# yuanzhi-zhu/DiffPIR

Measured on AMD Instinct MI355X. Metric: restored images/sec @100 NFE, 256x256, higher is better.
Workload: dtype f32 (GEMMs as 3 x f16 MFMA on hi/lo-split fp32 operands, fp32 accumulate; exact-fp32-MFMA mode in alt_precision); 1 GPU; configs[1]: ffhq topology 256x256 deblur (61x61 Gaussian PSF), 100 NFE, batch 16/GPU, device Philox noise, hipGraph=on; global_batch=16, nfe=100, collective=none

## Files before the change

diffpir_amd/_lib.py:

```python
from __future__ import annotations

import ctypes as C
import os

_HERE = os.path.dirname(os.path.abspath(__file__))
LIB_PATH = os.environ.get("DIFFPIR_LIB") or os.path.join(_HERE, "csrc", "libdiffpir_hip.so")
ABI_VERSION = 2



class UNetDesc(C.Structure):
    _fields_ = [("image_size", C.c_int32), ("in_channels", C.c_int32), ("model_channels", C.c_int32),
                ("out_channels", C.c_int32), ("num_res_blocks", C.c_int32), ("num_head_channels", C.c_int32),
                ("n_channel_mult", C.c_int32), ("channel_mult", C.c_float * 8),
                ("n_attention_ds", C.c_int32), ("attention_ds", C.c_int32 * 8), ("num_classes", C.c_int32)]


class Tensor(C.Structure):
    _fields_ = [("name", C.c_char_p), ("data", C.c_void_p), ("ndim", C.c_int32), ("shape", C.c_int64 * 4)]


class Step(C.Structure):
    _fields_ = [("t", C.c_int32), ("last", C.c_int32), ("c1", C.c_float), ("c2", C.c_float), ("tau", C.c_float),
                ("sa_t", C.c_float), ("s1m_t", C.c_float), ("sa_p", C.c_float),
# ... 164 lines not shown

DEBUG_LIB_PATH = os.path.join(_HERE, "csrc", "libdiffpir_dbg.so")
_dbg = None


def load_debug():
    global _dbg
    if _dbg is not None:
        return _dbg
    load()
    if not os.path.exists(DEBUG_LIB_PATH):
        raise EngineLibraryError(f"{DEBUG_LIB_PATH} not found: `make -C diffpir_amd/csrc` builds it next to the product library")
    d = C.CDLL(DEBUG_LIB_PATH)
    d.dpir_debug_conv_bench.argtypes = [C.c_void_p] + [C.c_int] * 10 + [C.POINTER(C.c_double)]
    d.dpir_debug_conv7_emit_supported.argtypes = [C.c_void_p] + [C.c_int] * 4 + [C.POINTER(C.c_int)]
    d.dpir_debug_victim.argtypes = [C.c_void_p, C.c_int, C.c_int, C.c_int, C.c_longlong, C.c_int, C.POINTER(C.c_ulonglong)]
    d.dpir_debug_victim_alu.argtypes = [C.c_void_p, C.c_int, C.c_int, C.c_int, C.c_int, C.POINTER(C.c_ulonglong)]
    for fn in (d.dpir_debug_victim_fft_pk, d.dpir_debug_victim_fft_nopk):
        fn.argtypes = [C.c_void_p, C.c_int, C.c_int, C.c_int, C.POINTER(C.c_ulonglong)]
    d.dpir_debug_conv7_check.argtypes = [C.c_void_p] + [C.c_int] * 10 + [C.POINTER(C.c_double), C.POINTER(C.c_double), C.POINTER(C.c_ulonglong),
                                                                        C.POINTER(C.c_float), C.POINTER(C.c_int)]
    d.dpir_debug_conv5_layer.argtypes = [C.c_void_p] + [C.c_int] * 7 + [C.c_void_p] * 7 + [C.POINTER(C.c_int)]
    d.dpir_debug_conv5_layer.restype = C.c_int
    d.dpir_debug_conv3_layer.argtypes = [C.c_void_p, C.POINTER(Conv3Desc)]
    d.dpir_debug_conv3_layer.restype = C.c_int
    d.dpir_debug_conv9_layer.argtypes = [C.c_void_p, C.POINTER(Conv9Desc)]
    d.dpir_debug_conv9_layer.restype = C.c_int
    d.dpir_debug_conv_up_layer.argtypes = [C.c_void_p, C.POINTER(ConvUpDesc)]
    d.dpir_debug_conv_up_layer.restype = C.c_int
    d.dpir_debug_conv_up_counts.argtypes = [C.POINTER(C.c_longlong), C.POINTER(C.c_longlong)]
    d.dpir_debug_conv_up_counts.restype = None
    d.dpir_debug_attention.argtypes = [C.c_void_p, C.POINTER(AttentionDesc)]
    d.dpir_debug_attention.restype = C.c_int
    d.dpir_debug_groupnorm.argtypes = [C.c_void_p, C.POINTER(GroupNormDesc)]
    d.dpir_debug_groupnorm.restype = C.c_int
    for n in ("dpir_debug_conv_bench", "dpir_debug_victim", "dpir_debug_victim_alu", "dpir_debug_victim_fft_pk", "dpir_debug_victim_fft_nopk",
              "dpir_debug_conv7_check"):
        getattr(d, n).restype = C.c_int
    _dbg = d
    return d


def load():
    global _lib
    if _lib is not None:
        return _lib
# ... 24 lines not shown
```

diffpir_amd/csrc/common.h:

```cpp
#pragma once
#include <hip/hip_runtime.h>
#include <stdint.h>
#include <stdio.h>
#include <string>
#include <vector>
#include <map>
#include <memory>
#include <mutex>

#include "../../include/diffpir_engine.h"

namespace dpir {

struct Status {
    int code = DPIR_OK;
    std::string msg;
    bool ok() const { return code == DPIR_OK; }
};

#define DPIR_HIP(expr)                                                                         \
    do {                                                                                       \
        hipError_t _e = (expr);                                                                \
        if (_e != hipSuccess) {                                                                \
            char _b[512];                                                                      \
// ... 126 lines not shown
    const struct Conv6Emit* emit = nullptr;
};
bool conv7_emit_supported(int B, int Cout, int H, int W);
bool conv6_supported(int H, int W);
int conv6_stat_slots(int H, int W);
Status launch_conv6(hipStream_t s, const Conv6Args& a, int* stat_kind_out = nullptr, PendingConv* pend_out = nullptr, int* kernel_out = nullptr);
Status launch_conv6_resolve(hipStream_t s, const PendingConv& p);
float pack_weights_conv6(const float* w_oihw, int cout, int cin, std::vector<uint16_t>& out);
struct Conv5Args {
    CatSrc src; const float4* prm = nullptr;
    const void* w16 = nullptr; float w16_scale = 1.f;
    const float* bias = nullptr; float* out = nullptr; const float* res = nullptr;
    int B = 0, Cout = 0, H = 0, W = 0;
    unsigned long long* range_ctr = nullptr;
    bool x1 = false;
    const float4* emit_prm = nullptr; void* emit_hi = nullptr; void* emit_lo = nullptr;
    const float* out_scale_dev = nullptr;
    int force_tile = 0;
};
constexpr int kConv5EmitMaxC = 384;
bool conv5_supported(int B, int Cout, int H, int W, bool has_prm = false);
bool conv5_small_supported(int B, int ca, int cb, int Cout, int H, int W, bool has_prm = false);
Status launch_conv5(hipStream_t s, const Conv5Args& a);
float pack_weights_f16x3_1x1(const float* w_oi, int cout, int cin, std::vector<uint16_t>& out);
struct Conv8Args {
    const float* x = nullptr;
    const float4* prm = nullptr;
    const void* w = nullptr; float w_scale = 1.f;
    const float* bias = nullptr; float* out = nullptr;
    int B = 0, C = 0, Cout = 0, H = 0, W = 0;
    unsigned long long* range_ctr = nullptr;
    bool x1 = false;
    bool silu = true;
};
bool conv8_supported(int B, int C, int Cout, int H, int W);
Status launch_conv8(hipStream_t s, const Conv8Args& a);
float pack_weights_conv8(const float* w_oihw, int cout, int cin, std::vector<uint16_t>& out);
Status launch_gn_stats(hipStream_t s, CatSrc src, int B, int HW, double2* part);
struct GnStatSrc { const float2* slots = nullptr; int nslots = 0; const double2* part = nullptr; int c = 0; };
Status launch_gn_prm(hipStream_t s, GnStatSrc sa, GnStatSrc sb, int HW, const float* gamma, const float* beta,
                     const float* film, int film_stride, int film_off, int B, int C, bool silu, float4* prm,
                     const StepDev* fstep = nullptr, int frows = 0, float2* stats_out = nullptr);
Status launch_time_embed(hipStream_t s, const int* t_dev, const int* y_dev, const float* freqs, const float* w0, const float* b0,
                         const float* w2, const float* b2, const float* label_emb, int B, int mc, float* tmp, float* semb);
Status launch_rows_gemv(hipStream_t s, const float* W, const float* bias, const float* x, int B, int R, int K, float* out);

// ... 4 lines not shown
```

diffpir_amd/csrc/conv5.hip:

```cpp
#include "common.h"
#include "lds_dma.h"
#include <vector>
#include <stdlib.h>

namespace dpir {

typedef float floatx16 __attribute__((ext_vector_type(16)));
typedef _Float16 half8 __attribute__((ext_vector_type(8)));

struct Conv5K {
    const float* sa; const float* sb; int ca, cb;
    unsigned bytes_a, bytes_b, bytes_w, bytes_prm;
    const float4* prm;
    const char* w16; const float* bias; float* out; const float* res;
    int B, Cout, HW;
    int n_chunks, n_co_blocks;
    int n_wblocks;
    int n_tiles, pair_xcd;
    long long total_px;
    float out_scale;
    const float* out_scale_dev;
    unsigned long long* range_ctr;
    const float4* eprm; _Float16* ehi; _Float16* elo; int eC8;
};


__device__ __forceinline__ float gn_apply(float v, const float4 m, bool silu) {
    float t = (v - m.x) * m.y + m.z;
    if (silu) t = t * __builtin_amdgcn_rcpf(1.0f + __builtin_amdgcn_exp2f(t * -1.4426950408889634f));
    return t;
}

template <bool HAS_PRM, bool X1, bool EMIT, int WCO, int WPX, int TPX>
__device__ __forceinline__ bool conv5_chunk(const float* __restrict__ xs, const half8* __restrict__ wh, const float4* __restrict__ ps,
                                            const float4* __restrict__ eprm, const int (&pxl)[WPX], const int (&pimg)[WPX], bool silu, bool emit_wg,
                                            _Float16* __restrict__ ehi, _Float16* __restrict__ elo, const size_t (&eoff)[WPX], size_t echunk,
                                            floatx16 (&acc)[WCO][WPX]) {
    const half8* wl = wh + 2 * (32 * WCO);
    bool bad = false;
    half8 bh[WPX], bl[WPX];
#pragma unroll
    for (int j = 0; j < WPX; ++j) {
        float v[8];
#pragma unroll
        for (int jj = 0; jj < 8; ++jj) v[jj] = xs[jj * TPX + pxl[j]];
        if (HAS_PRM) {
#pragma unroll
            for (int jj = 0; jj < 8; ++jj) v[jj] = gn_apply(v[jj], ps[pimg[j] * 16 + jj], silu);
        }
        if (EMIT) {
            if (emit_wg) {
                half8 eh, el;
#pragma unroll
                for (int jj = 0; jj < 8; ++jj) {
                    float t = gn_apply(v[jj], eprm[jj], silu);
                    bad |= !(fabsf(t) <= 65000.f);
                    t = fminf(fmaxf(t, -65000.f), 65000.f);
                    const _Float16 hh = (_Float16)t;
                    eh[jj] = hh;
                    el[jj] = (_Float16)(t - (float)hh);
                }
                const size_t eo = (eoff[j] + echunk) * 8;
                *reinterpret_cast<half8*>(ehi + eo) = eh;
                if (!X1) *reinterpret_cast<half8*>(elo + eo) = el;
            }
        }
#pragma unroll
        for (int jj = 0; jj < 8; ++jj) {
            bad |= !(fabsf(v[jj]) <= 65000.f);
            float x = fminf(fmaxf(v[jj], -65000.f), 65000.f);
            _Float16 hh = (_Float16)x;
            bh[j][jj] = hh;
            if (!X1) bl[j][jj] = (_Float16)(x - (float)hh);
        }
    }
    half8 ah[WCO], al[WCO];
#pragma unroll
    for (int i = 0; i < WCO; ++i) { ah[i] = wh[i * 32]; if (!X1) al[i] = wl[i * 32]; }
    if (!X1) {
#pragma unroll
        for (int i = 0; i < WCO; ++i)
#pragma unroll
            for (int j = 0; j < WPX; ++j)
                acc[i][j] = __builtin_amdgcn_mfma_f32_32x32x16_f16(al[i], bh[j], acc[i][j], 0, 0, 0);
#pragma unroll
        for (int i = 0; i < WCO; ++i)
#pragma unroll
            for (int j = 0; j < WPX; ++j)
                acc[i][j] = __builtin_amdgcn_mfma_f32_32x32x16_f16(ah[i], bl[j], acc[i][j], 0, 0, 0);
    }
#pragma unroll
    for (int i = 0; i < WCO; ++i)
#pragma unroll
        for (int j = 0; j < WPX; ++j)
            acc[i][j] = __builtin_amdgcn_mfma_f32_32x32x16_f16(ah[i], bh[j], acc[i][j], 0, 0, 0);
    return bad;
}

template <bool HAS_PRM, bool X1, bool EMIT, int WCO, int WPX, int NST>
__device__ __forceinline__ void conv5_body(const Conv5K p) {
    static_assert(!(HAS_PRM && EMIT), "the emitting variant multiplies the raw input");
    static_assert(!EMIT || (WCO == 4 && WPX == 2 && NST == 3), "planes are emitted by the 128 x 256 tile only");
    static_assert((WPX == 1 || WPX == 2) && (WCO == 2 || WCO == 4) && NST >= 3 && NST <= 4, "tile / ring shapes the DMA split is written for");
#if defined(__HIP_DEVICE_COMPILE__)
    constexpr int TCO = 32 * WCO, TPX = 128 * WPX;
    constexpr int XBYTES = 16 * TPX * 4;
    constexpr int WBYTES = TCO * 64;
    constexpr int PBYTES = HAS_PRM ? 1024 : 0;
    constexpr int STAGE = XBYTES + WBYTES + PBYTES;
    constexpr int NSTORE = EMIT ? (X1 ? WPX : 2 * WPX) : 0;
    __shared__ __attribute__((aligned(16))) char smem5[NST * STAGE + 512 + (EMIT ? kConv5EmitMaxC * 16 : 0)];
    float* bias_sh = reinterpret_cast<float*>(smem5 + NST * STAGE);
    float4* eprm_sh = reinterpret_cast<float4*>(smem5 + NST * STAGE + 512);

    const int tid = threadIdx.x;
    const int lane = tid & 63;
    const int wave = __builtin_amdgcn_readfirstlane(tid >> 6);
    const int l31 = lane & 31;
    const int half = lane >> 5;
    const int bid = blockIdx.x;
    int co_blk, tile;
    if (p.pair_xcd) {
        const int t = bid >> 3;
        co_blk = t % p.n_co_blocks;
// ... 10 lines not shown
    const int n_tile = px0 / HW;
    const bool emit_wg = EMIT && co_blk == 0;
    const bool prm_wave = HAS_PRM && wave == 0;

    const __amdgpu_buffer_rsrc_t rs_a = rsrc_uniform(p.sa, p.bytes_a);
    const __amdgpu_buffer_rsrc_t rs_b = rsrc_uniform(p.sb ? p.sb : p.sa, p.sb ? p.bytes_b : 0u);
    const __amdgpu_buffer_rsrc_t rs_w = rsrc_uniform(p.w16, p.bytes_w);
    const __amdgpu_buffer_rsrc_t rs_p = rsrc_uniform(HAS_PRM ? (const void*)p.prm : (const void*)p.w16, HAS_PRM ? p.bytes_prm : 0u);
    constexpr int RPI = 256 / TPX, LPR = 64 / RPI;
    constexpr int XPW = 4 / RPI;
    constexpr int WPW = WBYTES / 1024 / 4;
    const int lr = lane / LPR;
    const int gq = px0 + 4 * (lane % LPR);
    const bool q_ok = gq < total_px;
    const int qn = q_ok ? gq / HW : 0;
    const int qp = q_ok ? gq - qn * HW : 0;
    const unsigned voffA = q_ok ? (unsigned)(((size_t)qn * p.ca * HW + (size_t)lr * HW + qp) * 4) : kOutOfRange;
    const unsigned voffB = q_ok ? (unsigned)(((size_t)qn * p.cb * HW + (size_t)lr * HW + qp) * 4) : kOutOfRange;
    const unsigned lane16 = (unsigned)lane * 16u;
    const unsigned voffP = (HAS_PRM && n_tile + (lane >> 4) < p.B) ? (unsigned)(((size_t)(n_tile + (lane >> 4)) * C + (lane & 15)) * 16) : kOutOfRange;

    auto issue_dma = [&](int chunk, int st) __attribute__((always_inline)) {
        char* stage = smem5 + st * STAGE;
#pragma unroll
        for (int u = 0; u < XPW; ++u) {
            const int cc = wave * XPW + u;
            const int c = chunk * 16 + cc * RPI;
            char* dst = stage + cc * 1024;
            if (c < p.ca) BLDS6(rs_a, dst, (RPI == 1 || c + lr < p.ca) ? voffA : kOutOfRange, (unsigned)c * (unsigned)HW * 4u);
            else BLDS6(rs_b, dst, c + lr < C ? voffB : kOutOfRange, (unsigned)(c - p.ca) * (unsigned)HW * 4u);
        }
        constexpr int WPLANE = TCO * 16;
        const unsigned wsoff = TCO == 128 ? (unsigned)(chunk * p.n_co_blocks + co_blk) * 8192u
                                          : (unsigned)(chunk * p.n_wblocks + (co_blk >> 1)) * 8192u + (unsigned)(co_blk & 1) * (unsigned)WPLANE;
#pragma unroll
        for (int u = 0; u < WPW; ++u) {
            const int piece = wave * WPW + u;
            const int pb = piece * 1024;
            BLDS6(rs_w, stage + XBYTES + pb, lane16 + (pb / WPLANE) * 2048 + pb % WPLANE, wsoff);
        }
        if (prm_wave) BLDS6(rs_p, stage + XBYTES + WBYTES, voffP, (unsigned)chunk * 256u);
    };

    int pxl[WPX]; int pimg[WPX];
    size_t eoff[WPX];
#pragma unroll
    for (int j = 0; j < WPX; ++j) {
        pxl[j] = wave * (32 * WPX) + j * 32 + l31;
        const int g = px0 + pxl[j];
        const int pn = g < total_px ? g / HW : n_tile;
        pimg[j] = pn - n_tile;
        eoff[j] = EMIT ? ((size_t)pn * p.eC8 + half) * HW + (size_t)(g - pn * HW) : 0;
    }

    floatx16 acc[WCO][WPX];
#pragma unroll
    for (int i = 0; i < WCO; ++i)
#pragma unroll
        for (int j = 0; j < WPX; ++j)
#pragma unroll
            for (int r = 0; r < 16; ++r) acc[i][j][r] = 0.f;

    bool bad = false;
    bool silu = false;
    if (EMIT) {
        for (int c = tid; c < C; c += 256) eprm_sh[c] = p.eprm[(size_t)n_tile * C + c];
        silu = __builtin_amdgcn_readfirstlane(p.eprm[0].w != 0.f ? 1 : 0) != 0;
    }
    if (HAS_PRM) silu = __builtin_amdgcn_readfirstlane(p.prm[0].w != 0.f ? 1 : 0) != 0;
    if (tid < TCO) bias_sh[tid] = co_blk * TCO + tid < p.Cout ? p.bias[co_blk * TCO + tid] : 0.f;
    __builtin_amdgcn_sched_barrier(0);
    issue_dma(0, 0);
    if (p.n_chunks > 1) issue_dma(1, 1);
    if (NST > 3 && p.n_chunks > 2) issue_dma(2, 2);
    int st = 0;
    for (int chunk = 0; chunk < p.n_chunks; ++chunk) {
        constexpr int NDMA = XPW + WPW;
        __builtin_amdgcn_sched_barrier(0);
        if (chunk + 1 >= p.n_chunks) wait_vmcnt<0>();
        else if (NST > 3 && chunk + 2 < p.n_chunks) { if (prm_wave) wait_vmcnt<2 * NDMA + 2>(); else wait_vmcnt<2 * NDMA>(); }
        else if (emit_wg && chunk > 0) wait_vmcnt<NDMA + NSTORE>();
        else if (prm_wave) wait_vmcnt<NDMA + 1>();
        else wait_vmcnt<NDMA>();
        barrier_lds_only();
        if (chunk + NST - 1 < p.n_chunks) issue_dma(chunk + NST - 1, st == 0 ? NST - 1 : st - 1);
        __builtin_amdgcn_sched_barrier(0);

        const char* stage = smem5 + st * STAGE;
        bad |= conv5_chunk<HAS_PRM, X1, EMIT, WCO, WPX, TPX>(reinterpret_cast<const float*>(stage) + (8 * half) * TPX,
                                              reinterpret_cast<const half8*>(stage + XBYTES) + half * TCO + l31,
                                              reinterpret_cast<const float4*>(stage + XBYTES + WBYTES) + 8 * half,
                                              eprm_sh + chunk * 16 + 8 * half, pxl, pimg, silu, emit_wg,
                                              p.ehi, p.elo, eoff, (size_t)chunk * 2 * HW, acc);
        st = st == NST - 1 ? 0 : st + 1;
    }

    {
        const unsigned long long m = __ballot(bad);
        if (m != 0ull && p.range_ctr && lane == __builtin_ctzll(m)) atomicAdd(p.range_ctr, (unsigned long long)__builtin_popcountll(m));
    }
    __syncthreads();
    constexpr int SROW = 32 * WPX + 4;
    static_assert(4 * 32 * SROW * 4 <= NST * STAGE, "epilogue slabs alias the ring");
    constexpr int L4 = 8 * WPX;
    constexpr int NPS = 32 / (64 / L4);
    float* slab = reinterpret_cast<float*>(smem5) + wave * (32 * SROW);
    const int row_l = lane / L4, c4 = lane % L4;
    const int g4 = px0 + wave * (32 * WPX) + 4 * c4;
    const bool ok4 = g4 < total_px;
    const int n4 = ok4 ? g4 / HW : 0;
    const size_t base4 = (size_t)n4 * p.Cout * HW + (size_t)(g4 - n4 * HW);
    const int co0 = co_blk * TCO;
    const float osc = p.out_scale_dev ? p.out_scale * p.out_scale_dev[0] : p.out_scale;
#pragma unroll
    for (int i = 0; i < WCO; ++i) {
#pragma unroll
        for (int j = 0; j < WPX; ++j)
// ... 9 lines not shown
            }
            wait_vmcnt<0>();
        }
#pragma unroll
        for (int ps = 0; ps < NPS; ++ps) {
            const int row = ps * (64 / L4) + row_l;
            const int co = co0 + i * 32 + row;
            const float4 a4 = *reinterpret_cast<const float4*>(slab + row * SROW + 4 * c4);
            const float bz = bias_sh[i * 32 + row];
            if (ok4 && co < p.Cout) {
                float4 v = make_float4(a4.x * osc + bz, a4.y * osc + bz, a4.z * osc + bz, a4.w * osc + bz);
                if (p.res) v = make_float4(rr[ps].x + v.x, rr[ps].y + v.y, rr[ps].z + v.z, rr[ps].w + v.w);
                *reinterpret_cast<float4*>(p.out + base4 + (size_t)co * HW) = v;
            }
        }
    }
#endif
}

template <bool HAS_PRM, bool X1, bool EMIT>
__global__ __launch_bounds__(256, 2) void conv5_mfma_kernel(Conv5K p) { conv5_body<HAS_PRM, X1, EMIT, 4, 2, 3>(p); }
template <bool HAS_PRM, bool X1>
__global__ __launch_bounds__(256, 2) void conv5_small_mfma_kernel(Conv5K p) { conv5_body<HAS_PRM, X1, false, 2, 1, 4>(p); }

static bool conv5_shape_ok(int H, int W, bool has_prm) {
    if ((H * W) % 4) return false;
    return !(has_prm && (H * W) % 64);
}

bool conv5_supported(int B, int Cout, int H, int W, bool has_prm) {
    const long long px = (long long)B * H * W;
    if (!conv5_shape_ok(H, W, has_prm)) return false;
    return ((px + 255) / 256) * ((Cout + 127) / 128) >= 32;
}

static bool conv5_small_enabled() {
    static const bool on = !(getenv("DPIR_CONV5_SMALL") && atoi(getenv("DPIR_CONV5_SMALL")) == 0);
    return on;
}
static long long conv5_small_below() {
    static const long long v = getenv("DPIR_CONV5_SMALL_BELOW") ? atoll(getenv("DPIR_CONV5_SMALL_BELOW")) : 512;
    return v;
}
static bool conv5_small_shape_ok(int ca, int cb, int H, int W, bool has_prm) {
    return conv5_shape_ok(H, W, has_prm) && !(cb > 0 && ca % 4);
}

bool conv5_small_supported(int B, int ca, int cb, int Cout, int H, int W, bool has_prm) {
    const long long px = (long long)B * H * W;
    if (!conv5_small_enabled() || !conv5_small_shape_ok(ca, cb, H, W, has_prm)) return false;
    if (((px + 255) / 256) * ((Cout + 127) / 128) >= conv5_small_below()) return false;
    return ((px + 127) / 128) * ((Cout + 63) / 64) >= 32;
}

Status launch_conv5(hipStream_t s, const Conv5Args& a) {
    const int ca = a.src.ca, cb = a.src.b ? a.src.cb : 0;
    const bool has_prm = a.prm != nullptr;
    bool small;
    if (a.force_tile) {
        small = a.force_tile == 2;
        if (small ? (!conv5_small_shape_ok(ca, cb, a.H, a.W, has_prm) || a.emit_hi) : !conv5_shape_ok(a.H, a.W, has_prm))
            return Status{DPIR_ERR_UNSUPPORTED, "conv5: shape not tiled"};
    } else {
        small = !a.emit_hi && conv5_small_supported(a.B, ca, cb, a.Cout, a.H, a.W, has_prm);
        if (!small && !conv5_supported(a.B, a.Cout, a.H, a.W, has_prm)) return Status{DPIR_ERR_UNSUPPORTED, "conv5: shape not tiled"};
// ... 9 lines not shown
    k.n_wblocks = (a.Cout + 127) / 128;
    k.total_px = (long long)a.B * a.H * a.W;
    if (k.total_px >= (1ll << 31) - 256) return invalid("conv5: more than 2^31 pixels in the batch");
    const unsigned long long ba = (unsigned long long)k.total_px * k.ca * 4, bb = (unsigned long long)k.total_px * k.cb * 4;
    const unsigned long long bw = (unsigned long long)k.n_chunks * k.n_wblocks * 8192, bp = (unsigned long long)a.B * C * 16;
    if (ba >= (1ull << 32) || bb >= (1ull << 32) || bw >= (1ull << 32))
        return invalid("conv5: an input tensor exceeds the 4 GiB buffer-descriptor range; reduce the batch");
    k.bytes_a = (unsigned)ba; k.bytes_b = (unsigned)bb; k.bytes_w = (unsigned)bw; k.bytes_prm = (unsigned)bp;
    if (a.prm && C % 16) return invalid("conv5: the GroupNorm variant needs a multiple of 16 input channels");
    k.out_scale = 1.0f / a.w16_scale;
    k.out_scale_dev = a.out_scale_dev;
    k.range_ctr = a.range_ctr;
    k.eprm = a.emit_prm; k.ehi = reinterpret_cast<_Float16*>(a.emit_hi); k.elo = reinterpret_cast<_Float16*>(a.emit_lo);
    k.eC8 = 2 * k.n_chunks;
    k.n_tiles = (int)((k.total_px + tpx - 1) / tpx);
    static const bool pair_env = !(getenv("DPIR_CONV5_PAIR") && atoi(getenv("DPIR_CONV5_PAIR")) == 0);
    k.pair_xcd = pair_env && k.n_co_blocks > 1 ? 1 : 0;
    const unsigned blocks = k.pair_xcd ? (unsigned)((k.n_tiles + 7) / 8 * 8 * k.n_co_blocks) : (unsigned)(k.n_tiles * k.n_co_blocks);
    if (a.emit_hi) {
        if (a.prm || !a.emit_prm || (!a.x1 && !a.emit_lo)) return invalid("conv5: the plane-emitting variant takes the raw input and a GroupNorm table for the planes");
        if ((a.H * a.W) % 256 || C % 16 || C > kConv5EmitMaxC) return invalid("conv5: the plane-emitting variant needs H*W % 256 == 0 and a multiple of 16, at most 384, input channels");
        if (a.x1) hipLaunchKernelGGL((conv5_mfma_kernel<false, true, true>), dim3(blocks), dim3(256), 0, s, k);
        else hipLaunchKernelGGL((conv5_mfma_kernel<false, false, true>), dim3(blocks), dim3(256), 0, s, k);
    } else if (small) {
        if (a.x1) {
            if (a.prm) hipLaunchKernelGGL((conv5_small_mfma_kernel<true, true>), dim3(blocks), dim3(256), 0, s, k);
            else hipLaunchKernelGGL((conv5_small_mfma_kernel<false, true>), dim3(blocks), dim3(256), 0, s, k);
        } else if (a.prm) hipLaunchKernelGGL((conv5_small_mfma_kernel<true, false>), dim3(blocks), dim3(256), 0, s, k);
        else hipLaunchKernelGGL((conv5_small_mfma_kernel<false, false>), dim3(blocks), dim3(256), 0, s, k);
    } else if (a.x1) {
        if (a.prm) hipLaunchKernelGGL((conv5_mfma_kernel<true, true, false>), dim3(blocks), dim3(256), 0, s, k);
        else hipLaunchKernelGGL((conv5_mfma_kernel<false, true, false>), dim3(blocks), dim3(256), 0, s, k);
    } else if (a.prm) hipLaunchKernelGGL((conv5_mfma_kernel<true, false, false>), dim3(blocks), dim3(256), 0, s, k);
    else hipLaunchKernelGGL((conv5_mfma_kernel<false, false, false>), dim3(blocks), dim3(256), 0, s, k);
    DPIR_HIP(hipGetLastError());
    return Status{};
}

float pack_weights_f16x3_1x1(const float* w, int cout, int cin, std::vector<uint16_t>& out) {
    const int chunks = (cin + 15) / 16, cblocks = (cout + 127) / 128;
    float mx = 0.f;
    for (size_t i = 0; i < (size_t)cout * cin; ++i) mx = fmaxf(mx, fabsf(w[i]));
    float scale = 1.0f;
    if (mx > 0.f) scale = exp2f(floorf(log2f(1024.0f / mx)));
    while (mx * scale >= 1024.0f) scale *= 0.5f;
    const size_t plane = (size_t)2 * 128 * 8;
// ... 22 lines not shown
```

diffpir_amd/csrc/dbg_conv.hip:

```cpp
#include "engine.h"
#include "conv6_params.h"
#include "conv9.h"
#include "conv_up.h"
#include "../../include/diffpir_debug.h"
#include <string.h>
#include <vector>
using namespace dpir;
static int fail(dpir_engine* e, const Status& s) {
    if (e) e->last_error = s.msg;
    return s.code;
}
#define API_TRY(e, expr)                          \
    do {                                          \
        Status _s = (expr);                       \
        if (!_s.ok()) return fail((e), _s);       \
    } while (0)
#define API_HIP(e, expr)                                                                  \
    do {                                                                                  \
        hipError_t _h = (expr);                                                           \
        if (_h != hipSuccess)                                                             \
            return fail((e), Status{DPIR_ERR_HIP, std::string(#expr) + ": " + hipGetErrorString(_h)}); \
    } while (0)

__global__ void dbg_bitdiff_kernel(const float* a, const float* b, size_t n, unsigned long long* out) {
// ... 171 lines not shown
    }
    unsigned long long h[2] = {0, 0};
    API_HIP(e, hipMemcpyAsync(h, cmp, 16, hipMemcpyDeviceToHost, e->stream));
    API_HIP(e, hipStreamSynchronize(e->stream));
    *mismatches_out = h[0];
    const unsigned mb = (unsigned)h[1];
    *maxdiff_out = __builtin_bit_cast(float, mb);
    hipEvent_t e0, e1, e2;
    API_HIP(e, hipEventCreate(&e0)); API_HIP(e, hipEventCreate(&e1)); API_HIP(e, hipEventCreate(&e2));
    for (int i = 0; i < 3; ++i) { API_TRY(e, launch_conv6(e->stream, a6, &k6, &pend)); API_TRY(e, launch_conv7(e->stream, k, blocks * S, x1 != 0)); }
    API_HIP(e, hipEventRecord(e0, e->stream));
    for (int i = 0; i < iters; ++i) API_TRY(e, launch_conv6(e->stream, a6, &k6, &pend));
    API_HIP(e, hipEventRecord(e1, e->stream));
    for (int i = 0; i < iters; ++i) API_TRY(e, launch_conv7(e->stream, k, blocks * S, x1 != 0));
    API_HIP(e, hipEventRecord(e2, e->stream));
    API_HIP(e, hipEventSynchronize(e2));
    float m6 = 0, m7 = 0;
    API_HIP(e, hipEventElapsedTime(&m6, e0, e1)); API_HIP(e, hipEventElapsedTime(&m7, e1, e2));
    (void)hipEventDestroy(e0); (void)hipEventDestroy(e1); (void)hipEventDestroy(e2);
    *ms6_out = m6 / iters; *ms7_out = m7 / iters;
    return DPIR_OK;
}

int dpir_debug_conv5_layer(dpir_engine* e, int B, int ca, int cb, int Cout, int H, int W, int tile, const float* xa, const float* xb,
                           const float* w, const float* bias, const float* prm, const float* res, float* out, int* path_out) {
    if (!e || !xa || !w || !bias || !out || !path_out || B <= 0 || ca <= 0 || cb < 0 || (cb > 0 && !xb) || Cout <= 0 || tile < 0 || tile > 2) return DPIR_ERR_INVALID;
    if (e->precision == 0) return fail(e, invalid("conv5 layer: the engine is in f32 mode"));
    (void)hipSetDevice(e->device);
    const int C = ca + cb, HW = H * W;
    const size_t na = (size_t)B * ca * HW, nb = (size_t)B * cb * HW, no = (size_t)B * Cout * HW;
    float *dxa = nullptr, *dxb = nullptr, *dbias = nullptr, *dout = nullptr, *dres = nullptr, *dw = nullptr, *partial = nullptr; float4* dprm = nullptr;
    API_TRY(e, e->ws.getT("c5#xa", na, &dxa));
    API_TRY(e, e->ws.getT("c5#xb", nb + 1, &dxb));
    API_TRY(e, e->ws.getT("c5#b", (size_t)round_up(Cout, 64), &dbias));
    API_TRY(e, e->ws.getT("c5#o", no, &dout));
    API_TRY(e, e->ws.getT("c5#res", no, &dres));
    API_TRY(e, e->ws.getT("c5#prm", (size_t)B * C, &dprm));
    API_HIP(e, hipMemcpy(dxa, xa, na * 4, hipMemcpyHostToDevice));
    if (cb) API_HIP(e, hipMemcpy(dxb, xb, nb * 4, hipMemcpyHostToDevice));
    API_HIP(e, hipMemset(dbias, 0, (size_t)round_up(Cout, 64) * 4));
    API_HIP(e, hipMemcpy(dbias, bias, (size_t)Cout * 4, hipMemcpyHostToDevice));
    if (prm) API_HIP(e, hipMemcpy(dprm, prm, (size_t)B * C * 16, hipMemcpyHostToDevice));
    if (res) API_HIP(e, hipMemcpy(dres, res, no * 4, hipMemcpyHostToDevice));
    API_HIP(e, hipMemset(dout, 0xFF, no * 4));
    std::vector<uint16_t> w16v;
    const float w16_scale = pack_weights_f16x3_1x1(w, Cout, C, w16v);
    void* wp = nullptr;
    API_TRY(e, e->ws.get("c5#w16", w16v.size() * 2, &wp));
    API_HIP(e, hipMemcpy(wp, w16v.data(), w16v.size() * 2, hipMemcpyHostToDevice));
    const bool has_prm = prm != nullptr;
    const bool use5 = !(has_prm && C % 16) && (tile != 0 || conv5_supported(B, Cout, H, W, has_prm) || conv5_small_supported(B, ca, cb, Cout, H, W, has_prm));
    Status st;
    if (use5) {
        Conv5Args a5;
        a5.src = CatSrc{dxa, ca, cb ? dxb : nullptr, cb}; a5.prm = has_prm ? dprm : nullptr; a5.w16 = wp; a5.w16_scale = w16_scale;
        a5.bias = dbias; a5.out = dout; a5.res = res ? dres : nullptr; a5.B = B; a5.Cout = Cout; a5.H = H; a5.W = W;
        a5.x1 = e->precision == 2; a5.force_tile = tile;
        *path_out = tile ? tile : (conv5_small_supported(B, ca, cb, Cout, H, W, has_prm) ? 2 : 1);
        st = launch_conv5(e->stream, a5);
    } else {
        const int coutp = round_up(Cout, 64), cinp = round_up(C, 16);
        std::vector<float> packed((size_t)cinp * coutp, 0.f);
        for (int co = 0; co < Cout; ++co)
            for (int ci = 0; ci < C; ++ci) packed[(size_t)ci * coutp + co] = w[(size_t)co * C + ci];
        API_TRY(e, e->ws.getT("c5#w", packed.size(), &dw));
        API_HIP(e, hipMemcpy(dw, packed.data(), packed.size() * 4, hipMemcpyHostToDevice));
        API_TRY(e, e->ws.getT("conv#partial", (size_t)16 * 1024 * 1024, &partial));
        ConvArgs a;
        a.src.a = dxa; a.src.ca = ca; a.src.b = cb ? dxb : nullptr; a.src.cb = cb; a.src.Hs = H; a.src.Ws = W; a.src.mode = 0;
        a.src.prm = has_prm ? dprm : nullptr;
        a.w = dw; a.bias = dbias; a.out = dout; a.res = res ? dres : nullptr; a.res_mode = 0;
        a.B = B; a.Cin = C; a.Cout = Cout; a.CoutP = coutp; a.H = H; a.W = W; a.ks = 1;
        a.partial = partial; a.partial_capacity = (size_t)16 * 1024 * 1024;
        *path_out = 0;
        st = launch_conv(e->stream, a);
    }
    API_TRY(e, st);
    API_HIP(e, hipStreamSynchronize(e->stream));
    API_HIP(e, hipMemcpy(out, dout, no * 4, hipMemcpyDeviceToHost));
    return DPIR_OK;
}

int dpir_debug_conv3_layer(dpir_engine* e, dpir_debug_conv3_desc* d) {
    if (!e || !d) return DPIR_ERR_INVALID;
    d->path_out = -1; d->ksplit_out = 0; d->stat_kind_out = 0;
    const int B = d->B, ca = d->ca, cb = d->cb, Cout = d->Cout, H = d->H, W = d->W, mode = d->mode, C = ca + cb;
    if (!d->xa || !d->w || !d->bias || !d->out || B <= 0 || ca <= 0 || cb < 0 || (cb > 0 && !d->xb) || Cout <= 0 || H <= 0 || W <= 0 || mode < 0 || mode > 2 ||
        d->res_mode < -1 || d->res_mode > 2 || (d->res_mode >= 0 && !d->res) || d->prologue < 0 || d->prologue > 2 ||
        (d->route != 0 && d->route != 6 && d->route != 7 && d->route != 8))
        return fail(e, invalid("conv3 layer: bad descriptor"));
    if (d->prologue == 1 && !d->prm) return fail(e, invalid("conv3 layer: prologue 1 needs the table"));
    if (d->prologue == 2 && (!d->gamma || !d->beta)) return fail(e, invalid("conv3 layer: prologue 2 needs gamma and beta"));
    if (mode == 1 && ((H | W) & 1)) return fail(e, invalid("conv3 layer: a nearest-up source needs an even output size"));
    if (d->res_mode == 1 && ((H | W) & 1)) return fail(e, invalid("conv3 layer: a half-resolution residual needs an even output size"));
    if (d->defer && (!d->split || (d->route != 0 && d->route != 7) || !d->gamma2 || !d->beta2 || !d->w2 || !d->bias2 || !d->out2 || d->Cout2 <= 0))
        return fail(e, invalid("conv3 layer: defer needs split, route 0 or 7 and the second stage's operands"));
    (void)hipSetDevice(e->device);
    const int Hs = mode == 1 ? H / 2 : (mode == 2 ? H * 2 : H), Ws = mode == 1 ? W / 2 : (mode == 2 ? W * 2 : W);
    const size_t HWs = (size_t)Hs * Ws, HW = (size_t)H * W;
    const size_t na = (size_t)B * ca * HWs, nb = (size_t)B * cb * HWs, no = (size_t)B * Cout * HW;
    const size_t nres = d->res_mode == 1 ? no / 4 : (d->res_mode == 2 ? no * 4 : no);
    const int coutp = round_up(Cout, 64);
// ... 444 lines not shown
```

include/diffpir_debug.h:

```cpp
#ifndef DIFFPIR_DEBUG_H
#define DIFFPIR_DEBUG_H
#include "diffpir_engine.h"
#ifdef __cplusplus
extern "C" {
#endif
int dpir_debug_conv_bench(dpir_engine* e, int B, int Cin, int Cout, int H, int W, int ks, int mode, int with_prm,
                          int dbg, int iters, double* ms_out);
int dpir_debug_victim(dpir_engine* e, int lds_bytes, int threads, int blocks, long long spin_ticks, int iters, unsigned long long* bad_out);
int dpir_debug_victim_alu(dpir_engine* e, int mode, int blocks, int iters_in_kernel, int launches, unsigned long long* bad_out);
int dpir_debug_victim_fft_pk(dpir_engine* e, int blocks, int iters_in_kernel, int launches, unsigned long long* bad_out);
int dpir_debug_victim_fft_nopk(dpir_engine* e, int blocks, int iters_in_kernel, int launches, unsigned long long* bad_out);
int dpir_debug_conv7_check(dpir_engine* e, int B, int Cin, int Cout, int H, int W, int res_mode, int x1, int split, int scaled, int iters,
                           double* ms6_out, double* ms7_out, unsigned long long* mismatches_out, float* maxdiff_out, int* ksplit_out);
int dpir_debug_conv7_emit_supported(dpir_engine* e, int B, int Cout, int H, int W, int* capacity_out);
int dpir_debug_conv5_layer(dpir_engine* e, int B, int ca, int cb, int Cout, int H, int W, int tile, const float* xa, const float* xb,
                           const float* w, const float* bias, const float* prm, const float* res, float* out, int* path_out);
typedef struct dpir_debug_conv3_desc {
    int32_t B, ca, cb, Cout, H, W, mode, res_mode, scaled, prologue, route, split, defer, Cout2;
    const float *xa, *xb, *w, *bias, *res, *prm, *gamma, *beta, *film, *gamma2, *beta2, *w2, *bias2;
    float* out; double* stat_out; float* out2;
    int32_t stat_kind_out, path_out, ksplit_out, reserved;
} dpir_debug_conv3_desc;
int dpir_debug_conv3_layer(dpir_engine* e, dpir_debug_conv3_desc* d);
typedef struct dpir_debug_conv9_desc {
    int32_t B, Cin, Cout, H, W, res_mode, hop, Cout2;
    const float *x, *w, *bias, *res, *prm, *gamma2, *beta2, *film2, *w2, *bias2;
    float* out; double* stat_out; float* out2;
    int32_t ran_out, iters;
    double ms_out;
} dpir_debug_conv9_desc;
int dpir_debug_conv9_layer(dpir_engine* e, dpir_debug_conv9_desc* d);
typedef struct dpir_debug_conv_up_desc {
    int32_t B, Cin, Cout, Hs, Ws, hop, force_hop, Cout2, route, reserved;
    const float *x, *w, *bias, *res, *prm, *gamma2, *beta2, *film2, *w2, *bias2;
    float* out; double* stat_out; float* out2;
    int32_t ran_out, iters;
    double ms_out;
} dpir_debug_conv_up_desc;
int dpir_debug_conv_up_layer(dpir_engine* e, dpir_debug_conv_up_desc* d);
// ... 21 lines not shown
```

Before: 9.150 images/s.

## Add software-pipelined conv5 small-tile kernel overlapping MFMA with next chunk's split

Adds a pipelined variant of the small-tile (2x1, 4-stage) conv5 kernel. It keeps four DMA stages in flight and double-buffers the f16 hi/lo operands, so the MFMAs for the current chunk run while the next chunk's LDS loads and hi/lo split are in progress. Interleaving is guided by sched_group_barrier. It also simplifies DMA address computation when channels align to 16, and it is on by default for eligible shapes. In exchange, register pressure is higher and the schedule is more complex; env and debug overrides allow falling back.

```diff
diff --git a/diffpir_amd/_lib.py b/diffpir_amd/_lib.py
--- a/diffpir_amd/_lib.py
+++ b/diffpir_amd/_lib.py
@@ -210,6 +210,10 @@
                                                                         C.POINTER(C.c_float), C.POINTER(C.c_int)]
     d.dpir_debug_conv5_layer.argtypes = [C.c_void_p] + [C.c_int] * 7 + [C.c_void_p] * 7 + [C.POINTER(C.c_int)]
     d.dpir_debug_conv5_layer.restype = C.c_int
+    d.dpir_debug_conv5_layer_range.argtypes = d.dpir_debug_conv5_layer.argtypes + [C.POINTER(C.c_ulonglong)]
+    d.dpir_debug_conv5_layer_range.restype = C.c_int
+    d.dpir_debug_set_conv5_small_pipe.argtypes = [C.c_int]
+    d.dpir_debug_set_conv5_small_pipe.restype = C.c_int
     d.dpir_debug_conv3_layer.argtypes = [C.c_void_p, C.POINTER(Conv3Desc)]
     d.dpir_debug_conv3_layer.restype = C.c_int
     d.dpir_debug_conv9_layer.argtypes = [C.c_void_p, C.POINTER(Conv9Desc)]
diff --git a/diffpir_amd/csrc/common.h b/diffpir_amd/csrc/common.h
--- a/diffpir_amd/csrc/common.h
+++ b/diffpir_amd/csrc/common.h
@@ -172,6 +172,7 @@
 bool conv5_supported(int B, int Cout, int H, int W, bool has_prm = false);
 bool conv5_small_supported(int B, int ca, int cb, int Cout, int H, int W, bool has_prm = false);
 Status launch_conv5(hipStream_t s, const Conv5Args& a);
+void conv5_small_pipe_override(int v);
 float pack_weights_f16x3_1x1(const float* w_oi, int cout, int cin, std::vector<uint16_t>& out);
 struct Conv8Args {
     const float* x = nullptr;
diff --git a/diffpir_amd/csrc/conv5.hip b/diffpir_amd/csrc/conv5.hip
--- a/diffpir_amd/csrc/conv5.hip
+++ b/diffpir_amd/csrc/conv5.hip
@@ -1,5 +1,6 @@
 #include "common.h"
 #include "lds_dma.h"
+#include <type_traits>
 #include <vector>
 #include <stdlib.h>
 
@@ -31,75 +32,98 @@
     return t;
 }
 
+template <int TPX>
+__device__ __forceinline__ void conv5_load_b(const float* __restrict__ xs, int pxl, float (&v)[8]) {
+#pragma unroll
+    for (int jj = 0; jj < 8; ++jj) v[jj] = xs[jj * TPX + pxl];
+}
+
+template <bool HAS_PRM, bool X1, bool EMIT>
+__device__ __forceinline__ bool conv5_split(float (&v)[8], const float4* __restrict__ ps, const float4* __restrict__ eprm, int pimg, bool silu, bool emit_wg,
+                                            _Float16* __restrict__ ehi, _Float16* __restrict__ elo, size_t eo, half8& bh, half8& bl) {
+    bool bad = false;
+    if (HAS_PRM) {
+#pragma unroll
+        for (int jj = 0; jj < 8; ++jj) v[jj] = gn_apply(v[jj], ps[pimg * 16 + jj], silu);
+    }
+    if (EMIT) {
+        if (emit_wg) {
+            half8 eh, el;
+#pragma unroll
+            for (int jj = 0; jj < 8; ++jj) {
+                float t = gn_apply(v[jj], eprm[jj], silu);
+                bad |= !(fabsf(t) <= 65000.f);
+                t = fminf(fmaxf(t, -65000.f), 65000.f);
+                const _Float16 hh = (_Float16)t;
+                eh[jj] = hh;
+                el[jj] = (_Float16)(t - (float)hh);
+            }
+            *reinterpret_cast<half8*>(ehi + eo) = eh;
+            if (!X1) *reinterpret_cast<half8*>(elo + eo) = el;
+        }
+    }
+#pragma unroll
+    for (int jj = 0; jj < 8; ++jj) {
+        bad |= !(fabsf(v[jj]) <= 65000.f);
+        float x = fminf(fmaxf(v[jj], -65000.f), 65000.f);
+        _Float16 hh = (_Float16)x;
+        bh[jj] = hh;
+        if (!X1) bl[jj] = (_Float16)(x - (float)hh);
+    }
+    return bad;
+}
+
+template <bool X1, int WCO>
+__device__ __forceinline__ void conv5_load_a(const half8* __restrict__ wh, half8 (&ah)[WCO], half8 (&al)[WCO]) {
+    const half8* wl = wh + 2 * (32 * WCO);
+#pragma unroll
+    for (int i = 0; i < WCO; ++i) { ah[i] = wh[i * 32]; if (!X1) al[i] = wl[i * 32]; }
+}
+
+template <bool X1, int WCO, int WPX>
+__device__ __forceinline__ void conv5_multiply(const half8 (&bh)[WPX], const half8 (&bl)[WPX], const half8 (&ah)[WCO], const half8 (&al)[WCO],
+                                               floatx16 (&acc)[WCO][WPX]) {
+    if (!X1) {
+#pragma unroll
+        for (int i = 0; i < WCO; ++i)
+#pragma unroll
+            for (int j = 0; j < WPX; ++j)
+                acc[i][j] = __builtin_amdgcn_mfma_f32_32x32x16_f16(al[i], bh[j], acc[i][j], 0, 0, 0);
+#pragma unroll
+        for (int i = 0; i < WCO; ++i)
+#pragma unroll
+            for (int j = 0; j < WPX; ++j)
+                acc[i][j] = __builtin_amdgcn_mfma_f32_32x32x16_f16(ah[i], bl[j], acc[i][j], 0, 0, 0);
+    }
+#pragma unroll
+    for (int i = 0; i < WCO; ++i)
+#pragma unroll
+        for (int j = 0; j < WPX; ++j)
+            acc[i][j] = __builtin_amdgcn_mfma_f32_32x32x16_f16(ah[i], bh[j], acc[i][j], 0, 0, 0);
+}
+
 template <bool HAS_PRM, bool X1, bool EMIT, int WCO, int WPX, int TPX>
 __device__ __forceinline__ bool conv5_chunk(const float* __restrict__ xs, const half8* __restrict__ wh, const float4* __restrict__ ps,
                                             const float4* __restrict__ eprm, const int (&pxl)[WPX], const int (&pimg)[WPX], bool silu, bool emit_wg,
                                             _Float16* __restrict__ ehi, _Float16* __restrict__ elo, const size_t (&eoff)[WPX], size_t echunk,
                                             floatx16 (&acc)[WCO][WPX]) {
-    const half8* wl = wh + 2 * (32 * WCO);
     bool bad = false;
-    half8 bh[WPX], bl[WPX];
+    half8 bh[WPX], bl[WPX], ah[WCO], al[WCO];
 #pragma unroll
     for (int j = 0; j < WPX; ++j) {
         float v[8];
-#pragma unroll
-        for (int jj = 0; jj < 8; ++jj) v[jj] = xs[jj * TPX + pxl[j]];
-        if (HAS_PRM) {
-#pragma unroll
-            for (int jj = 0; jj < 8; ++jj) v[jj] = gn_apply(v[jj], ps[pimg[j] * 16 + jj], silu);
-        }
-        if (EMIT) {
-            if (emit_wg) {
-                half8 eh, el;
-#pragma unroll
-                for (int jj = 0; jj < 8; ++jj) {
-                    float t = gn_apply(v[jj], eprm[jj], silu);
-                    bad |= !(fabsf(t) <= 65000.f);
-                    t = fminf(fmaxf(t, -65000.f), 65000.f);
-                    const _Float16 hh = (_Float16)t;
-                    eh[jj] = hh;
-                    el[jj] = (_Float16)(t - (float)hh);
-                }
-                const size_t eo = (eoff[j] + echunk) * 8;
-                *reinterpret_cast<half8*>(ehi + eo) = eh;
-                if (!X1) *reinterpret_cast<half8*>(elo + eo) = el;
-            }
-        }
-#pragma unroll
-        for (int jj = 0; jj < 8; ++jj) {
-            bad |= !(fabsf(v[jj]) <= 65000.f);
-            float x = fminf(fmaxf(v[jj], -65000.f), 65000.f);
-            _Float16 hh = (_Float16)x;
-            bh[j][jj] = hh;
-            if (!X1) bl[j][jj] = (_Float16)(x - (float)hh);
-        }
-    }
-    half8 ah[WCO], al[WCO];
-#pragma unroll
-    for (int i = 0; i < WCO; ++i) { ah[i] = wh[i * 32]; if (!X1) al[i] = wl[i * 32]; }
-    if (!X1) {
-#pragma unroll
-        for (int i = 0; i < WCO; ++i)
-#pragma unroll
-            for (int j = 0; j < WPX; ++j)
-                acc[i][j] = __builtin_amdgcn_mfma_f32_32x32x16_f16(al[i], bh[j], acc[i][j], 0, 0, 0);
-#pragma unroll
-        for (int i = 0; i < WCO; ++i)
-#pragma unroll
-            for (int j = 0; j < WPX; ++j)
-                acc[i][j] = __builtin_amdgcn_mfma_f32_32x32x16_f16(ah[i], bl[j], acc[i][j], 0, 0, 0);
-    }
-#pragma unroll
-    for (int i = 0; i < WCO; ++i)
-#pragma unroll
-        for (int j = 0; j < WPX; ++j)
-            acc[i][j] = __builtin_amdgcn_mfma_f32_32x32x16_f16(ah[i], bh[j], acc[i][j], 0, 0, 0);
+        conv5_load_b<TPX>(xs, pxl[j], v);
+        bad |= conv5_split<HAS_PRM, X1, EMIT>(v, ps, eprm, pimg[j], silu, emit_wg, ehi, elo, (eoff[j] + echunk) * 8, bh[j], bl[j]);
+    }
+    conv5_load_a<X1, WCO>(wh, ah, al);
+    conv5_multiply<X1, WCO, WPX>(bh, bl, ah, al, acc);
     return bad;
 }
 
-template <bool HAS_PRM, bool X1, bool EMIT, int WCO, int WPX, int NST>
+template <bool HAS_PRM, bool X1, bool EMIT, int WCO, int WPX, int NST, bool PIPE = false>
 __device__ __forceinline__ void conv5_body(const Conv5K p) {
     static_assert(!(HAS_PRM && EMIT), "the emitting variant multiplies the raw input");
+    static_assert(!PIPE || (!EMIT && WCO == 2 && WPX == 1 && NST == 4), "the pipelined loop is written for the small tile");
     static_assert(!EMIT || (WCO == 4 && WPX == 2 && NST == 3), "planes are emitted by the 128 x 256 tile only");
     static_assert((WPX == 1 || WPX == 2) && (WCO == 2 || WCO == 4) && NST >= 3 && NST <= 4, "tile / ring shapes the DMA split is written for");
 #if defined(__HIP_DEVICE_COMPILE__)
@@ -156,13 +180,23 @@
 
     auto issue_dma = [&](int chunk, int st) __attribute__((always_inline)) {
         char* stage = smem5 + st * STAGE;
-#pragma unroll
-        for (int u = 0; u < XPW; ++u) {
-            const int cc = wave * XPW + u;
-            const int c = chunk * 16 + cc * RPI;
-            char* dst = stage + cc * 1024;
-            if (c < p.ca) BLDS6(rs_a, dst, (RPI == 1 || c + lr < p.ca) ? voffA : kOutOfRange, (unsigned)c * (unsigned)HW * 4u);
-            else BLDS6(rs_b, dst, c + lr < C ? voffB : kOutOfRange, (unsigned)(c - p.ca) * (unsigned)HW * 4u);
+        if constexpr (PIPE) {
+            const int c0 = chunk * 16;
+            const bool from_a = c0 < p.ca;
+            const __amdgpu_buffer_rsrc_t rs = from_a ? rs_a : rs_b;
+            const unsigned voff = from_a ? voffA : voffB;
+            const unsigned soff = ((unsigned)(from_a ? c0 : c0 - p.ca) + (unsigned)(wave * XPW * RPI)) * ((unsigned)HW * 4u);
+#pragma unroll
+            for (int u = 0; u < XPW; ++u) BLDS6(rs, stage + (wave * XPW + u) * 1024, voff, soff + (unsigned)(u * RPI) * ((unsigned)HW * 4u));
+        } else {
+#pragma unroll
+            for (int u = 0; u < XPW; ++u) {
+                const int cc = wave * XPW + u;
+                const int c = chunk * 16 + cc * RPI;
+                char* dst = stage + cc * 1024;
+                if (c < p.ca) BLDS6(rs_a, dst, (RPI == 1 || c + lr < p.ca) ? voffA : kOutOfRange, (unsigned)c * (unsigned)HW * 4u);
+                else BLDS6(rs_b, dst, c + lr < C ? voffB : kOutOfRange, (unsigned)(c - p.ca) * (unsigned)HW * 4u);
+            }
         }
         constexpr int WPLANE = TCO * 16;
         const unsigned wsoff = TCO == 128 ? (unsigned)(chunk * p.n_co_blocks + co_blk) * 8192u
@@ -204,29 +238,99 @@
     if (HAS_PRM) silu = __builtin_amdgcn_readfirstlane(p.prm[0].w != 0.f ? 1 : 0) != 0;
     if (tid < TCO) bias_sh[tid] = co_blk * TCO + tid < p.Cout ? p.bias[co_blk * TCO + tid] : 0.f;
     __builtin_amdgcn_sched_barrier(0);
-    issue_dma(0, 0);
-    if (p.n_chunks > 1) issue_dma(1, 1);
-    if (NST > 3 && p.n_chunks > 2) issue_dma(2, 2);
-    int st = 0;
-    for (int chunk = 0; chunk < p.n_chunks; ++chunk) {
+    if constexpr (PIPE) {
         constexpr int NDMA = XPW + WPW;
+        const int n = p.n_chunks;
+        auto wait_chunk = [&](int ahead) __attribute__((always_inline)) {
+            if (ahead >= 3) { if (prm_wave) wait_vmcnt<3 * NDMA + 3>(); else wait_vmcnt<3 * NDMA>(); }
+            else if (ahead == 2) { if (prm_wave) wait_vmcnt<2 * NDMA + 2>(); else wait_vmcnt<2 * NDMA>(); }
+            else if (ahead == 1) { if (prm_wave) wait_vmcnt<NDMA + 1>(); else wait_vmcnt<NDMA>(); }
+            else wait_vmcnt<0>();
+        };
+        auto load = [&](int st, float (&v)[8], half8 (&ah)[WCO], half8 (&al)[WCO]) __attribute__((always_inline)) {
+            const char* stage = smem5 + st * STAGE;
+            conv5_load_b<TPX>(reinterpret_cast<const float*>(stage) + (8 * half) * TPX, pxl[0], v);
+            conv5_load_a<X1, WCO>(reinterpret_cast<const half8*>(stage + XBYTES) + half * TCO + l31, ah, al);
+        };
+        auto split = [&](int st, float (&v)[8], half8& bh, half8& bl) __attribute__((always_inline)) {
+            return conv5_split<HAS_PRM, X1, false>(v, reinterpret_cast<const float4*>(smem5 + st * STAGE + XBYTES + WBYTES) + 8 * half, eprm_sh, pimg[0],
+                                                   silu, false, p.ehi, p.elo, 0, bh, bl);
+        };
+        half8 bh0[WPX], bl0[WPX], ah0[WCO], al0[WCO], bh1[WPX], bl1[WPX], ah1[WCO], al1[WCO];
+        auto step = [&](auto steady_c, int c, half8 (&bhc)[WPX], half8 (&blc)[WPX], half8 (&ahc)[WCO], half8 (&alc)[WCO],
+                        half8 (&bhn)[WPX], half8 (&bln)[WPX], half8 (&ahn)[WCO], half8 (&aln)[WCO]) __attribute__((always_inline)) {
+            constexpr bool STEADY = decltype(steady_c)::value;
+            if (STEADY || c + 1 < n) {
+                __builtin_amdgcn_sched_barrier(0);
+                wait_chunk(STEADY || n - 2 - c >= 2 ? 2 : n - 2 - c);
+                barrier_lds_only();
+                if (STEADY || c + NST < n) issue_dma(c + NST, c & (NST - 1));
+                __builtin_amdgcn_sched_barrier(0);
+                const int stn = (c + 1) & (NST - 1);
+                float v[8];
+                load(stn, v, ahn, aln);
+                __builtin_amdgcn_sched_barrier(0);
+                conv5_multiply<X1, WCO, WPX>(bhc, blc, ahc, alc, acc);
+                bad |= split(stn, v, bhn[0], bln[0]);
+                constexpr int NV = HAS_PRM ? 40 : 16;
+                __builtin_amdgcn_sched_group_barrier(0x8, WCO, 0);
+                if (!X1) {
+                    __builtin_amdgcn_sched_group_barrier(0x2, NV, 0);
+                    __builtin_amdgcn_sched_group_barrier(0x8, WCO, 0);
+                    __builtin_amdgcn_sched_group_barrier(0x2, NV, 0);
+                    __builtin_amdgcn_sched_group_barrier(0x8, WCO, 0);
+                }
+            } else {
+                conv5_multiply<X1, WCO, WPX>(bhc, blc, ahc, alc, acc);
+            }
+        };
+        issue_dma(0, 0);
+        if (n > 1) issue_dma(1, 1);
+        if (n > 2) issue_dma(2, 2);
+        if (n > 3) issue_dma(3, 3);
         __builtin_amdgcn_sched_barrier(0);
-        if (chunk + 1 >= p.n_chunks) wait_vmcnt<0>();
-        else if (NST > 3 && chunk + 2 < p.n_chunks) { if (prm_wave) wait_vmcnt<2 * NDMA + 2>(); else wait_vmcnt<2 * NDMA>(); }
-        else if (emit_wg && chunk > 0) wait_vmcnt<NDMA + NSTORE>();
-        else if (prm_wave) wait_vmcnt<NDMA + 1>();
-        else wait_vmcnt<NDMA>();
+        wait_chunk(n < NST ? n - 1 : NST - 1);
         barrier_lds_only();
-        if (chunk + NST - 1 < p.n_chunks) issue_dma(chunk + NST - 1, st == 0 ? NST - 1 : st - 1);
         __builtin_amdgcn_sched_barrier(0);
-
-        const char* stage = smem5 + st * STAGE;
-        bad |= conv5_chunk<HAS_PRM, X1, EMIT, WCO, WPX, TPX>(reinterpret_cast<const float*>(stage) + (8 * half) * TPX,
-                                              reinterpret_cast<const half8*>(stage + XBYTES) + half * TCO + l31,
-                                              reinterpret_cast<const float4*>(stage + XBYTES + WBYTES) + 8 * half,
-                                              eprm_sh + chunk * 16 + 8 * half, pxl, pimg, silu, emit_wg,
-                                              p.ehi, p.elo, eoff, (size_t)chunk * 2 * HW, acc);
-        st = st == NST - 1 ? 0 : st + 1;
+        {
+            float v[8];
+            load(0, v, ah0, al0);
+            bad |= split(0, v, bh0[0], bl0[0]);
+        }
+        int c = 0;
+        for (; c + NST + 1 < n; c += 2) {
+            step(std::true_type{}, c, bh0, bl0, ah0, al0, bh1, bl1, ah1, al1);
+            step(std::true_type{}, c + 1, bh1, bl1, ah1, al1, bh0, bl0, ah0, al0);
+        }
+        for (; c < n; c += 2) {
+            step(std::false_type{}, c, bh0, bl0, ah0, al0, bh1, bl1, ah1, al1);
+            if (c + 1 < n) step(std::false_type{}, c + 1, bh1, bl1, ah1, al1, bh0, bl0, ah0, al0);
+        }
+    } else {
+        issue_dma(0, 0);
+        if (p.n_chunks > 1) issue_dma(1, 1);
+        if (NST > 3 && p.n_chunks > 2) issue_dma(2, 2);
+        int st = 0;
+        for (int chunk = 0; chunk < p.n_chunks; ++chunk) {
+            constexpr int NDMA = XPW + WPW;
+            __builtin_amdgcn_sched_barrier(0);
+            if (chunk + 1 >= p.n_chunks) wait_vmcnt<0>();
+            else if (NST > 3 && chunk + 2 < p.n_chunks) { if (prm_wave) wait_vmcnt<2 * NDMA + 2>(); else wait_vmcnt<2 * NDMA>(); }
+            else if (emit_wg && chunk > 0) wait_vmcnt<NDMA + NSTORE>();
+            else if (prm_wave) wait_vmcnt<NDMA + 1>();
+            else wait_vmcnt<NDMA>();
+            barrier_lds_only();
+            if (chunk + NST - 1 < p.n_chunks) issue_dma(chunk + NST - 1, st == 0 ? NST - 1 : st - 1);
+            __builtin_amdgcn_sched_barrier(0);
+
+            const char* stage = smem5 + st * STAGE;
+            bad |= conv5_chunk<HAS_PRM, X1, EMIT, WCO, WPX, TPX>(reinterpret_cast<const float*>(stage) + (8 * half) * TPX,
+                                                  reinterpret_cast<const half8*>(stage + XBYTES) + half * TCO + l31,
+                                                  reinterpret_cast<const float4*>(stage + XBYTES + WBYTES) + 8 * half,
+                                                  eprm_sh + chunk * 16 + 8 * half, pxl, pimg, silu, emit_wg,
+                                                  p.ehi, p.elo, eoff, (size_t)chunk * 2 * HW, acc);
+            st = st == NST - 1 ? 0 : st + 1;
+        }
     }
 
     {
@@ -282,6 +386,8 @@
 __global__ __launch_bounds__(256, 2) void conv5_mfma_kernel(Conv5K p) { conv5_body<HAS_PRM, X1, EMIT, 4, 2, 3>(p); }
 template <bool HAS_PRM, bool X1>
 __global__ __launch_bounds__(256, 2) void conv5_small_mfma_kernel(Conv5K p) { conv5_body<HAS_PRM, X1, false, 2, 1, 4>(p); }
+template <bool HAS_PRM, bool X1>
+__global__ __launch_bounds__(256, 2) void conv5_small_pipe_kernel(Conv5K p) { conv5_body<HAS_PRM, X1, false, 2, 1, 4, true>(p); }
 
 static bool conv5_shape_ok(int H, int W, bool has_prm) {
     if ((H * W) % 4) return false;
@@ -301,6 +407,13 @@
 static long long conv5_small_below() {
     static const long long v = getenv("DPIR_CONV5_SMALL_BELOW") ? atoll(getenv("DPIR_CONV5_SMALL_BELOW")) : 512;
     return v;
+}
+static bool conv5_pipe_shape_ok(int ca, int cb) { return (ca + cb) % 16 == 0 && (cb == 0 || ca % 16 == 0); }
+static int g_conv5_pipe_override = -1;
+void conv5_small_pipe_override(int v) { g_conv5_pipe_override = v; }
+static bool conv5_small_pipe_enabled() {
+    static const bool on = !(getenv("DPIR_CONV5_SMALL_PIPE") && atoi(getenv("DPIR_CONV5_SMALL_PIPE")) == 0);
+    return g_conv5_pipe_override < 0 ? on : g_conv5_pipe_override != 0;
 }
 static bool conv5_small_shape_ok(int ca, int cb, int H, int W, bool has_prm) {
     return conv5_shape_ok(H, W, has_prm) && !(cb > 0 && ca % 4);
@@ -356,6 +469,12 @@
         if ((a.H * a.W) % 256 || C % 16 || C > kConv5EmitMaxC) return invalid("conv5: the plane-emitting variant needs H*W % 256 == 0 and a multiple of 16, at most 384, input channels");
         if (a.x1) hipLaunchKernelGGL((conv5_mfma_kernel<false, true, true>), dim3(blocks), dim3(256), 0, s, k);
         else hipLaunchKernelGGL((conv5_mfma_kernel<false, false, true>), dim3(blocks), dim3(256), 0, s, k);
+    } else if (small && conv5_pipe_shape_ok(ca, cb) && conv5_small_pipe_enabled()) {
+        if (a.x1) {
+            if (a.prm) hipLaunchKernelGGL((conv5_small_pipe_kernel<true, true>), dim3(blocks), dim3(256), 0, s, k);
+            else hipLaunchKernelGGL((conv5_small_pipe_kernel<false, true>), dim3(blocks), dim3(256), 0, s, k);
+        } else if (a.prm) hipLaunchKernelGGL((conv5_small_pipe_kernel<true, false>), dim3(blocks), dim3(256), 0, s, k);
+        else hipLaunchKernelGGL((conv5_small_pipe_kernel<false, false>), dim3(blocks), dim3(256), 0, s, k);
     } else if (small) {
         if (a.x1) {
             if (a.prm) hipLaunchKernelGGL((conv5_small_mfma_kernel<true, true>), dim3(blocks), dim3(256), 0, s, k);
diff --git a/diffpir_amd/csrc/dbg_conv.hip b/diffpir_amd/csrc/dbg_conv.hip
--- a/diffpir_amd/csrc/dbg_conv.hip
+++ b/diffpir_amd/csrc/dbg_conv.hip
@@ -217,8 +217,8 @@
     return DPIR_OK;
 }
 
-int dpir_debug_conv5_layer(dpir_engine* e, int B, int ca, int cb, int Cout, int H, int W, int tile, const float* xa, const float* xb,
-                           const float* w, const float* bias, const float* prm, const float* res, float* out, int* path_out) {
+static int conv5_layer(dpir_engine* e, int B, int ca, int cb, int Cout, int H, int W, int tile, const float* xa, const float* xb,
+                       const float* w, const float* bias, const float* prm, const float* res, float* out, int* path_out, unsigned long long* range_out) {
     if (!e || !xa || !w || !bias || !out || !path_out || B <= 0 || ca <= 0 || cb < 0 || (cb > 0 && !xb) || Cout <= 0 || tile < 0 || tile > 2) return DPIR_ERR_INVALID;
     if (e->precision == 0) return fail(e, invalid("conv5 layer: the engine is in f32 mode"));
     (void)hipSetDevice(e->device);
@@ -251,6 +251,10 @@
         a5.src = CatSrc{dxa, ca, cb ? dxb : nullptr, cb}; a5.prm = has_prm ? dprm : nullptr; a5.w16 = wp; a5.w16_scale = w16_scale;
         a5.bias = dbias; a5.out = dout; a5.res = res ? dres : nullptr; a5.B = B; a5.Cout = Cout; a5.H = H; a5.W = W;
         a5.x1 = e->precision == 2; a5.force_tile = tile;
+        if (range_out) {
+            API_HIP(e, hipMemsetAsync(e->range_ctr, 0, sizeof(unsigned long long), e->stream));
+            a5.range_ctr = e->range_ctr;
+        }
         *path_out = tile ? tile : (conv5_small_supported(B, ca, cb, Cout, H, W, has_prm) ? 2 : 1);
         st = launch_conv5(e->stream, a5);
     } else {
@@ -273,6 +277,28 @@
     API_TRY(e, st);
     API_HIP(e, hipStreamSynchronize(e->stream));
     API_HIP(e, hipMemcpy(out, dout, no * 4, hipMemcpyDeviceToHost));
+    if (range_out) {
+        *range_out = 0;
+        if (use5) {
+            API_HIP(e, hipMemcpy(range_out, e->range_ctr, sizeof(unsigned long long), hipMemcpyDeviceToHost));
+            API_HIP(e, hipMemset(e->range_ctr, 0, sizeof(unsigned long long)));
+        }
+    }
+    return DPIR_OK;
+}
+int dpir_debug_conv5_layer(dpir_engine* e, int B, int ca, int cb, int Cout, int H, int W, int tile, const float* xa, const float* xb,
+                           const float* w, const float* bias, const float* prm, const float* res, float* out, int* path_out) {
+    return conv5_layer(e, B, ca, cb, Cout, H, W, tile, xa, xb, w, bias, prm, res, out, path_out, nullptr);
+}
+int dpir_debug_conv5_layer_range(dpir_engine* e, int B, int ca, int cb, int Cout, int H, int W, int tile, const float* xa, const float* xb,
+                                 const float* w, const float* bias, const float* prm, const float* res, float* out, int* path_out,
+                                 unsigned long long* range_out) {
+    if (!range_out) return DPIR_ERR_INVALID;
+    return conv5_layer(e, B, ca, cb, Cout, H, W, tile, xa, xb, w, bias, prm, res, out, path_out, range_out);
+}
+int dpir_debug_set_conv5_small_pipe(int pipe) {
+    if (pipe < -1 || pipe > 1) return DPIR_ERR_INVALID;
+    conv5_small_pipe_override(pipe);
     return DPIR_OK;
 }
 
diff --git a/include/diffpir_debug.h b/include/diffpir_debug.h
--- a/include/diffpir_debug.h
+++ b/include/diffpir_debug.h
@@ -15,6 +15,10 @@
 int dpir_debug_conv7_emit_supported(dpir_engine* e, int B, int Cout, int H, int W, int* capacity_out);
 int dpir_debug_conv5_layer(dpir_engine* e, int B, int ca, int cb, int Cout, int H, int W, int tile, const float* xa, const float* xb,
                            const float* w, const float* bias, const float* prm, const float* res, float* out, int* path_out);
+int dpir_debug_conv5_layer_range(dpir_engine* e, int B, int ca, int cb, int Cout, int H, int W, int tile, const float* xa, const float* xb,
+                                 const float* w, const float* bias, const float* prm, const float* res, float* out, int* path_out,
+                                 unsigned long long* range_out);
+int dpir_debug_set_conv5_small_pipe(int pipe);
 typedef struct dpir_debug_conv3_desc {
     int32_t B, ca, cb, Cout, H, W, mode, res_mode, scaled, prologue, route, split, defer, Cout2;
     const float *xa, *xb, *w, *bias, *res, *prm, *gamma, *beta, *film, *gamma2, *beta2, *w2, *bias2;
```

After: 9.206 images/s, median of 6. Within noise of the previous version (+0.6%).
